# Enderdead/pyNeuralEMPC

Measured on AMD Instinct MI355X. Metric: nlp_callback_evals_per_sec (f + grad f + g + dense jac g), higher is better.
Workload: dtype f64; 1 GPU; configs[1] dims: 2x1 MLP(2x64), H=20, Euler(Discret), fp64; north_star batch=1024 per GPU; batch_per_gpu=1024, H=20, nx=2, nu=1, integrator=discret, n=60, m=40, row_kernel=mfma, parallelism=problem-sharded x1, clock=sustained (timed region after prime_ms of the same step)

## Files before the change

### pyneuralempc_amd/csrc/kernels_coopfx_impl.h

```cpp
#pragma once

#include "kernels_coop_impl.h"
#include "kernels_obj_impl.h"

#ifndef NEMPC_FX_ZERO_EARLY
#define NEMPC_FX_ZERO_EARLY 0
#endif

#ifdef NEMPC_STAMPS_NO_FX
#undef COOP_WGSTAMP
#undef COOP_WGSTAMP_REAL
#define COOP_WGSTAMP(p, i) do { } while (0)
#define COOP_WGSTAMP_REAL(p, i) do { } while (0)
#endif
#ifdef NEMPC_STAMPS_PRO
#define FX_STAMP_PASS(p, i) do { } while (0)
#define FX_STAMP_PRO(p, i) COOP_WGSTAMP(p, i)
#else
#define FX_STAMP_PASS(p, i) COOP_WGSTAMP(p, i)
#define FX_STAMP_PRO(p, i) do { } while (0)
#endif


namespace nempc {

template <typename T, int WP, int NH, int TPW, int NX, int NU>
struct FxLayout {
    static constexpr int MT = WP / 16;
    static constexpr int NIN = NX + NU;
    static constexpr int KS = (NIN + 3) / 4;
    static constexpr int NR = sizeof(T) == 8 ? (NIN + 3) / 4 : 4;
    static constexpr int NRO = sizeof(T) == 8 ? (NX + 3) / 4 : 4;
    static constexpr int JROW = NX * NIN;
    static constexpr int W0F = 0;
    static constexpr int SEED = W0F + KS * MT * 64;
    static constexpr int BIAS = SEED + NX * MT * 16;
    static constexpr int BIASL = BIAS + NH * MT * 16;
    static constexpr int P0 = BIASL + 16;
    static constexpr int SMALL_END = P0 + NIN * MT * 16;
    static constexpr int XH = TPW * MT * 256;
    static constexpr int X = (SMALL_END + 15) & ~15;
    static constexpr int PART = X + 2 * XH;
    static constexpr int PF_SZ = TPW * MT * NX * 16;
    static constexpr int PART_SZ = PF_SZ + NX * TPW * MT * NIN * 16;
    static constexpr int IN_TILE = 16 * (NIN + NX);
    static constexpr int IN = PART + PART_SZ;
    static constexpr int IN_SZ = (TPW * IN_TILE + 15) & ~15;
    static constexpr int TOTAL = IN + 2 * IN_SZ;
};

constexpr int FX_ZCOPY = 512;

struct FxArgs {
    const void* Z;
    const void* X0;
    const void* small;
    const void* wslice;
    int tiles_per_wg, tiles_rem;
    unsigned R;
    unsigned invH;
    int H, n, m;
    int ident;
    int box;
    int small_vecs;
    void* g;
    void* tiles;
    void* jac;
    void* f;
    void* grad;
    const void* P;
    int p_elems;
    int zp_max;
    long long* dbg;
    ObjOffsets oo;
    void* gn_hvals;
    const void* gn_sigma;
    const void* gn_w;
    const int32_t* gn_smap;
    const void* gn_objc;
    int gn_nnz, gn_n_orph;
    void* jac_sp;
    int sp_nnz;
};

constexpr int FX_ARGS_KERNARG_OFFSET = 64;
typedef const FxArgs __attribute__((address_space(4)))* FxArgsK;
__device__ __forceinline__ FxArgsK fx_late_args() {
    const char __attribute__((address_space(4)))* kp =
        (const char __attribute__((address_space(4)))*)__builtin_amdgcn_kernarg_segment_ptr();
    asm volatile("" : "+s"(kp));
    return (FxArgsK)(kp + FX_ARGS_KERNARG_OFFSET);
}

template <typename T, int WP, int NH, int TPW, int NX, int NU>
struct FxCtx {
    using L = FxLayout<T, WP, NH, TPW, NX, NU>;
    T* lds;
    const T* __restrict__ Z;
    const T* __restrict__ X0;
    unsigned R, invH;
    int H, n;
    bool rev;
    T* jac;
    bool box;
    long long* dbg;
};

template <typename T, int NT, int NTHREADS, int NCOL>
struct FxStage {
    static constexpr int ROWS = NT * 16;
    static constexpr int ITEMS = (NCOL * ROWS + NTHREADS - 1) / NTHREADS;
    T v[ITEMS];
};

template <typename T, int WP, int NH, int TPW, int NX, int NU, int NT>
__device__ __forceinline__ void fx_stage_load(const FxCtx<T, WP, NH, TPW, NX, NU>& cx, int t0, int tid,
                                              FxStage<T, NT, (WP / 16) * 64, NX + NU + NX>& sr) {
    constexpr int NIN = NX + NU, NCOL = NIN + NX, ROWS = NT * 16, NTHREADS = (WP / 16) * 64;
#pragma unroll
    for (int it = 0; it < FxStage<T, NT, NTHREADS, NCOL>::ITEMS; ++it) {
        const int item = tid + it * NTHREADS;
        const int col = item / ROWS, idx = item - col * ROWS;
        T v = T(0);
        const unsigned r = (unsigned)t0 * 16u + (unsigned)idx;
        if (col < NCOL && r < cx.R) {
            const unsigned b = cx.invH ? __umulhi(r, cx.invH) : r;
            const int t = (int)(r - b * (unsigned)cx.H);
            const T* z = cx.Z + (size_t)b * cx.n;
            if (col < NX) v = (t == 0) ? cx.X0[(size_t)b * NX + col] : z[(t - 1) * NX + col];
            else if (col < NIN) v = z[cx.H * NX + t * NU + (col - NX)];
            else v = z[t * NX + (col - NIN)];
        }
        sr.v[it] = v;
    }
}

template <typename T, int WP, int NH, int TPW, int NX, int NU, int NT>
__device__ __forceinline__ void fx_stage_store(T* in, int tid, const FxStage<T, NT, (WP / 16) * 64, NX + NU + NX>& sr) {
    constexpr int NIN = NX + NU, NCOL = NIN + NX, ROWS = NT * 16, NTHREADS = (WP / 16) * 64;
    using L = FxLayout<T, WP, NH, TPW, NX, NU>;
#pragma unroll
    for (int it = 0; it < FxStage<T, NT, NTHREADS, NCOL>::ITEMS; ++it) {
        const int item = tid + it * NTHREADS;
        const int col = item / ROWS, idx = item - col * ROWS;
        if (col < NCOL) {
            T* tile = in + (idx >> 4) * L::IN_TILE;
            if (col < NIN) tile[(idx & 15) * NIN + col] = sr.v[it];
            else tile[16 * NIN + (idx & 15) * NX + (col - NIN)] = sr.v[it];
        }
    }
}

__device__ __forceinline__ double fx_qsum(double s) {
    unsigned lo = (unsigned)__double2loint(s), hi = (unsigned)__double2hiint(s);
    auto l16 = __builtin_amdgcn_permlane16_swap(lo, lo, false, false);
    auto h16 = __builtin_amdgcn_permlane16_swap(hi, hi, false, false);
    s = __hiloint2double((int)h16[0], (int)l16[0]) + __hiloint2double((int)h16[1], (int)l16[1]);
    lo = (unsigned)__double2loint(s); hi = (unsigned)__double2hiint(s);
    auto l32 = __builtin_amdgcn_permlane32_swap(lo, lo, false, false);
    auto h32 = __builtin_amdgcn_permlane32_swap(hi, hi, false, false);
    return __hiloint2double((int)h32[0], (int)l32[0]) + __hiloint2double((int)h32[1], (int)l32[1]);
}
__device__ __forceinline__ float fx_qsum(float s) {
    unsigned v = __float_as_uint(s);
    auto a16 = __builtin_amdgcn_permlane16_swap(v, v, false, false);
    s = __uint_as_float(a16[0]) + __uint_as_float(a16[1]);
    v = __float_as_uint(s);
    auto a32 = __builtin_amdgcn_permlane32_swap(v, v, false, false);
// ... 3 lines not shown
__device__ __forceinline__ double fx_swap16_add(double a, double b) {
    auto l = __builtin_amdgcn_permlane16_swap((unsigned)__double2loint(a), (unsigned)__double2loint(b), false, false);
    auto h = __builtin_amdgcn_permlane16_swap((unsigned)__double2hiint(a), (unsigned)__double2hiint(b), false, false);
    return __hiloint2double((int)h[0], (int)l[0]) + __hiloint2double((int)h[1], (int)l[1]);
}
__device__ __forceinline__ double fx_swap32_add(double a, double b) {
    auto l = __builtin_amdgcn_permlane32_swap((unsigned)__double2loint(a), (unsigned)__double2loint(b), false, false);
    auto h = __builtin_amdgcn_permlane32_swap((unsigned)__double2hiint(a), (unsigned)__double2hiint(b), false, false);
    return __hiloint2double((int)h[0], (int)l[0]) + __hiloint2double((int)h[1], (int)l[1]);
}
__device__ __forceinline__ float fx_swap16_add(float a, float b) {
    auto v = __builtin_amdgcn_permlane16_swap(__float_as_uint(a), __float_as_uint(b), false, false);
    return __uint_as_float(v[0]) + __uint_as_float(v[1]);
}
__device__ __forceinline__ float fx_swap32_add(float a, float b) {
    auto v = __builtin_amdgcn_permlane32_swap(__float_as_uint(a), __float_as_uint(b), false, false);
    return __uint_as_float(v[0]) + __uint_as_float(v[1]);
}
template <typename T, int NV>
__device__ __forceinline__ void fx_rowsums_store(const T (&s)[NV], T* dst, int lane) {
    const int q = lane >> 4;
#pragma unroll
    for (int g = 0; g < NV / 4; ++g)
        dst[g * 64 + lane] = fx_swap32_add(fx_swap16_add(s[4 * g], s[4 * g + 1]), fx_swap16_add(s[4 * g + 2], s[4 * g + 3]));
    constexpr int G = NV / 4, REM = NV % 4;
    if constexpr (REM == 1) {
        const T v = fx_qsum(s[4 * G]);
        if (q == 0) dst[G * 64 + lane] = v;
    } else if constexpr (REM == 2) {
        const T p = fx_swap16_add(s[4 * G], s[4 * G + 1]);
        const T v = fx_swap32_add(p, p);
        if (q < 2) dst[G * 64 + lane] = v;
    } else if constexpr (REM == 3) {
        const T v = fx_swap32_add(fx_swap16_add(s[4 * G], s[4 * G + 1]), fx_swap16_add(s[4 * G + 2], s[4 * G + 2]));
        if (q < 3) dst[G * 64 + lane] = v;
    }
}

template <typename T, int NX, int NTHREADS>
__device__ __forceinline__ void fx_zero_rows(T* o_jac, unsigned r0, int nrows, int n, int H, unsigned invH, bool box, int tid) {
    constexpr int VEC = 16 / (int)sizeof(T);
    typedef T vecT __attribute__((ext_vector_type(VEC)));
    const vecT zero = {};
    const int nvec = n / VEC;
#if defined(NEMPC_EXP_NODENSE) || defined(NEMPC_EXP_NOZERO)
    const int drv = 0;
#else
    const int drv = nrows * NX;
#endif
    auto run = [&](const char* base, int nv) {
        const int full = nv / NTHREADS;
        const int voff = tid * 16;
        for (int k = 0; k < full; ++k) {
#ifdef NEMPC_STAMPS
            base = fx_uniform_ptr(base);
#endif
            asm volatile("global_store_dwordx4 %0, %1, %2 sc0 sc1\n\ts_nop 1" ::"v"(voff), "v"(zero), "s"(base) : "memory");
            base += NTHREADS * 16;
        }
#ifdef NEMPC_STAMPS
        base = fx_uniform_ptr(base);
#endif
        if (tid < nv - full * NTHREADS)
            asm volatile("global_store_dwordx4 %0, %1, %2 sc0 sc1\n\ts_nop 1" ::"v"(voff), "v"(zero), "s"(base) : "memory");
    };
    if (!box) {
        run(fx_uniform_ptr(reinterpret_cast<const char*>(o_jac) + (size_t)r0 * NX * (size_t)n * sizeof(T)), drv * nvec);
    } else {
        const int HNX = H * NX;
        for (int s0 = 0; s0 < drv;) {
            const unsigned r = r0 + (unsigned)(s0 / NX);
            const unsigned b = invH ? __umulhi(r, invH) : r;
            const int k = (int)(r - b * (unsigned)H) * NX;
            const int len = drv - s0 < HNX - k ? drv - s0 : HNX - k;
#pragma unroll
            for (int kind = 0; kind < 2; ++kind)
                run(fx_uniform_ptr(reinterpret_cast<const char*>(o_jac) +
                                   ((size_t)b * (2 * HNX) + (size_t)(kind * HNX + k)) * (size_t)n * sizeof(T)), len * nvec);
            s0 += len;
        }
    }
}

template <typename T, int WP, int NH, int TPW, int NX, int NU, int NT, bool FUSE, int ACT, bool GN = false>
__device__ __forceinline__ void fx_pass(const FxCtx<T, WP, NH, TPW, NX, NU>& cx, const CoopWeights<T, WP, NH>& W,
                                        const T* in, int t0, int tid, int& xsel,
                                        const FxStage<T, TPW, (WP / 16) * 64, NX + NU + NX>& nxt, bool has_next, T* in_next) {
    using Ops = MfmaOps<T>;
    using A = Act<T, ACT>;
    static_assert(ACT != NEMPC_ACT_RUNTIME, "the compiled-shape kernels take a compile-time activation");
    using V4 = typename Ops::V4;
    using L = FxLayout<T, WP, NH, TPW, NX, NU>;
    constexpr int MT = WP / 16, NTHREADS = MT * 64, NIN = NX + NU, KS = L::KS, JROW = L::JROW;
    const int lane = tid & 63, w = tid >> 6;
    const int c = lane & 15, q = lane >> 4;
    T* const lds = cx.lds;
    T* const PART = lds + L::PART;

    V4 a[NH][NT];
    {
        const T* bias = lds + L::BIAS + w * 16;
        V4 b0;
#pragma unroll
        for (int r = 0; r < 4; ++r) b0[r] = bias[r * 4 + q];
#pragma unroll
        for (int j = 0; j < NT; ++j) a[0][j] = b0;
#pragma unroll
        for (int ks = 0; ks < KS; ++ks) {
            const T wfrag = lds[L::W0F + (ks * MT + w) * 64 + lane];
            const int d = 4 * ks + q;
#pragma unroll
            for (int j = 0; j < NT; ++j) {
                const T v = d < NIN ? in[j * L::IN_TILE + c * NIN + d] : T(0);
                a[0][j] = Ops::mma(wfrag, v, a[0][j]);
            }
        }
#pragma unroll
        for (int j = 0; j < NT; ++j)
#pragma unroll
            for (int r = 0; r < 4; ++r) a[0][j][r] = A::f(a[0][j][r]);
    }
    FX_STAMP_PRO(cx.dbg, 10);
#if !NEMPC_FX_ZERO_EARLY
    if constexpr (FUSE) {
        if (cx.jac) {
            const unsigned r0 = (unsigned)t0 * 16u;
            const int nrows = r0 + (unsigned)NT * 16u <= cx.R ? NT * 16 : (int)(cx.R - r0);
            fx_zero_rows<T, NX, NTHREADS>(cx.jac, r0, nrows, cx.n, cx.H, cx.invH, cx.box, tid);
        }
    }
#endif
#pragma unroll
    for (int l = 1; l < NH; ++l) {
        T* X = lds + L::X + (xsel & 1) * L::XH;
        ++xsel;
#pragma unroll
        for (int j = 0; j < NT; ++j)
#pragma unroll
            for (int r = 0; r < 4; ++r) X[((j * MT + w) * 4 + r) * 64 + lane] = a[l - 1][j][r];
        lds_barrier();
        const T* bias = lds + L::BIAS + l * MT * 16 + w * 16;
        V4 b0;
#pragma unroll
        for (int r = 0; r < 4; ++r) b0[r] = bias[r * 4 + q];
#pragma unroll
        for (int j = 0; j < NT; ++j) a[l][j] = b0;
#pragma unroll
        for (int mt = 0; mt < MT; ++mt)
#pragma unroll
            for (int r = 0; r < 4; ++r)
#pragma unroll
                for (int j = 0; j < NT; ++j)
                    a[l][j] = Ops::mma(W.wf[l - 1][mt * 4 + r], X[((j * MT + mt) * 4 + r) * 64 + lane], a[l][j]);
#pragma unroll
        for (int j = 0; j < NT; ++j)
#pragma unroll
            for (int r = 0; r < 4; ++r) a[l][j][r] = A::f(a[l][j][r]);
    }
    FX_STAMP_PRO(cx.dbg, 11);
    V4 wl[NX];
#pragma unroll
    for (int k = 0; k < NX; ++k) {
        const T* seed = lds + L::SEED + k * MT * 16 + w * 16;
#pragma unroll
        for (int r = 0; r < 4; ++r) wl[k][r] = seed[r * 4 + q];
    }
    {
        T sv[NT * NX];
#pragma unroll
        for (int j = 0; j < NT; ++j)
#pragma unroll
            for (int k = 0; k < NX; ++k) {
                T v = a[NH - 1][j][0] * wl[k][0];
#pragma unroll
                for (int r = 1; r < 4; ++r) v = fma(a[NH - 1][j][r], wl[k][r], v);
                sv[j * NX + k] = v;
            }
        fx_rowsums_store<T, NT * NX>(sv, PART + w * (TPW * NX) * 16, lane);
    }
    FX_STAMP_PASS(cx.dbg, 5);
    T* const PJ = PART + L::PF_SZ;
    if (cx.rev) {
#pragma unroll
    for (int l = 0; l < NH; ++l)
#pragma unroll
        for (int j = 0; j < NT; ++j)
#pragma unroll
            for (int r = 0; r < 4; ++r) a[l][j][r] = A::d1(a[l][j][r]);

#pragma unroll
    for (int k = 0; k < NX; ++k) {
        V4 cv[NT];
#pragma unroll
        for (int j = 0; j < NT; ++j) cv[j] = wl[k] * a[NH - 1][j];
#pragma unroll
        for (int l = NH - 1; l >= 1; --l) {
            T* X = lds + L::X + (xsel & 1) * L::XH;
            ++xsel;
#pragma unroll
            for (int j = 0; j < NT; ++j)
#pragma unroll
                for (int r = 0; r < 4; ++r) X[((j * MT + w) * 4 + r) * 64 + lane] = cv[j][r];
            lds_barrier();
            V4 cn[NT];
#pragma unroll
// ... 144 lines not shown
            T f = lds[L::BIASL + rr * 4 + qq];
#pragma unroll
            for (int ww = 0; ww < MT; ++ww) f += PART[(ww * (TPW * NX) + j * NX + i) * 16 + cc];
            const T* tin = in + j * L::IN_TILE;
            const T xp = tin[cc * NIN + i];
            const T xt = tin[16 * NIN + cc * NX + i];
            const T phi = (a_ident ? xp : T(0)) + f;
            const unsigned b = cx.invH ? __umulhi(r, cx.invH) : r;
            const int t = (int)(r - b * (unsigned)cx.H);
            T* gp = o_g + (size_t)b * a_m + t * NX + i;
            gp[0] = phi - xt;
            if (a_box) gp[(size_t)cx.H * NX] = xt;
            if constexpr (FUSE) {
                if (o_jac || o_sp) {
                    const int n = cx.n;
                    T ts[NIN];
#pragma unroll
                    for (int d = 0; d < NIN; ++d) {
                        T v = T(0);
#pragma unroll
                        for (int ww = 0; ww < MT; ++ww) v += PJ[((i * MT + ww) * (TPW * NIN) + j * NIN + d) * 16 + cc];
                        if (a_ident && d == i) v += T(1);
                        ts[d] = v;
                    }
                    if (o_jac) {
                    if (o_tiles) {
#pragma unroll
                        for (int d = 0; d < NIN; ++d) o_tiles[(size_t)r * JROW + i * NIN + d] = ts[d];
                    }
                    T* const row = o_jac + ((size_t)b * a_m + (size_t)(t * NX + i)) * (size_t)n;
                    if (t >= 1) {
                        if constexpr (NX == 2 && sizeof(T) == 8) {
                            fx_store_wt2(row + (t - 1) * NX, ts[0], ts[1]);
                        } else {
#pragma unroll
                            for (int jj = 0; jj < NX; ++jj) fx_store_wt(row + (t - 1) * NX + jj, ts[jj]);
                        }
                    }
                    fx_store_wt(row + t * NX + i, T(-1));
#pragma unroll
                    for (int jj = 0; jj < NU; ++jj) fx_store_wt(row + cx.H * NX + t * NU + jj, ts[NX + jj]);
                    if (a_box) fx_store_wt(row + (size_t)cx.H * NX * (size_t)n + t * NX + i, T(1));
                    }
                    if (o_sp) {
                        constexpr int ROW0 = 1 + NU, ROWT = NX + 1 + NU;
                        T* const sp = o_sp + (size_t)b * sp_nnz;
                        if (t >= 1) {
                            T* const pc = sp + NX * ROW0 + ((t - 1) * NX + i) * ROWT;
                            if constexpr (NX == 2 && NU == 1 && sizeof(T) == 8) {
                                fx_store_wt2(pc, ts[0], ts[1]);
                                fx_store_wt2(pc + 2, T(-1), ts[2]);
                            } else {
#pragma unroll
                                for (int jj = 0; jj < NX; ++jj) pc[jj] = ts[jj];
                                pc[NX] = T(-1);
#pragma unroll
                                for (int jj = 0; jj < NU; ++jj) pc[NX + 1 + jj] = ts[NX + jj];
                            }
                        } else {
                            T* const pc = sp + i * ROW0;
                            if constexpr (NX == 2 && NU == 1 && sizeof(T) == 8) {
                                fx_store_wt2(pc, T(-1), ts[2]);
                            } else {
                                pc[0] = T(-1);
#pragma unroll
                                for (int jj = 0; jj < NU; ++jj) pc[1 + jj] = ts[NX + jj];
                            }
                        }
                        if (a_box) sp[NX * ROW0 + (cx.H - 1) * NX * ROWT + t * NX + i] = T(1);
                    }
                }
            }
        }
    }
    FX_STAMP_PASS(cx.dbg, 8);
    FX_STAMP_PASS(cx.dbg, 11);
    lds_barrier();
    FX_STAMP_PASS(cx.dbg, 12);
}

template <typename T, int WP, int NH, int TPW, int NX, int NU, bool FUSE, int ACT, bool GN = false>
__global__ __launch_bounds__((WP / 16) * 64, 2) void rows_coopfx_kernel(
    const void* pZ, const void* pX0, const void* psmall, const void* pwslice, const void* pP, unsigned ppack, unsigned pR,
    unsigned pinvH, int pH, void* pjac, FxArgs a) {
    struct {
        const void *Z, *X0, *small, *wslice, *P;
        int tiles_per_wg, tiles_rem, zp_max, H, n, p_elems;
        unsigned R, invH;
        ObjOffsets oo;
        long long* dbg;
    } pa;
    pa.Z = pZ; pa.X0 = pX0; pa.small = psmall; pa.wslice = pwslice; pa.P = pP;
    pa.tiles_per_wg = (int)(ppack & 0xffu); pa.tiles_rem = (int)((ppack >> 8) & 0x3ffu);
    pa.zp_max = (int)((ppack >> 18) & 0x3ffu);
#ifdef NEMPC_EXP_NOOBJ
    const bool want_obj = false;
#else
    const bool want_obj = ((ppack >> 28) & 3u) != 0;
#endif
    const bool want_rev = (ppack >> 30) & 1u;
    const bool has_box = (ppack >> 31) & 1u;
    pa.R = pR; pa.invH = pinvH; pa.H = pH; pa.n = pH * (NX + NU);
    pa.oo = obj_offsets(pH, NX, NU);
    pa.p_elems = FUSE ? pa.oo.total : 0;
#ifdef NEMPC_STAMPS
    pa.dbg = a.dbg;
#else
    pa.dbg = nullptr;
    (void)a;
#endif
    COOP_WGSTAMP(pa.dbg, 0);
#if defined(NEMPC_STAMPS) && !defined(NEMPC_STAMPS_NO_FX)
    if (pa.dbg && threadIdx.x == 0 && blockIdx.x < 4096)
        pa.dbg[1024 + blockIdx.x * 16 + 15] = ((long long)__builtin_amdgcn_s_getreg(63508) << 32) | (unsigned)__builtin_amdgcn_s_getreg(63492);
#endif
    using L = FxLayout<T, WP, NH, TPW, NX, NU>;
    constexpr int MT = WP / 16;
    constexpr int NTHREADS = MT * 64;
    constexpr int VEC = 16 / (int)sizeof(T);
    constexpr int NCOL = NX + NU + NX;
    typedef T vecT __attribute__((ext_vector_type(VEC)));
    extern __shared__ __attribute__((aligned(16))) unsigned char lds_raw[];
    T* lds = reinterpret_cast<T*>(lds_raw);

    const int tid = threadIdx.x;
    const int lane = tid & 63, w = tid >> 6;

    FxCtx<T, WP, NH, TPW, NX, NU> cx;
    cx.lds = lds;
    cx.Z = static_cast<const T*>(pa.Z);
    cx.X0 = static_cast<const T*>(pa.X0);
    cx.R = pa.R; cx.invH = pa.invH; cx.H = pa.H; cx.n = pa.n; cx.rev = want_rev;
    cx.jac = FUSE ? static_cast<T*>(pjac) : nullptr;
    cx.box = has_box;

    const int t_begin = blockIdx.x * pa.tiles_per_wg + ((int)blockIdx.x < pa.tiles_rem ? (int)blockIdx.x : pa.tiles_rem);
    const int t_end = t_begin + pa.tiles_per_wg + ((int)blockIdx.x < pa.tiles_rem ? 1 : 0);

    FxStage<T, TPW, NTHREADS, NCOL> sr;
    int t0 = t_begin;
    fx_stage_load<T, WP, NH, TPW, NX, NU, TPW>(cx, t0, tid, sr);
    FX_STAMP_PRO(pa.dbg, 1);
    constexpr int SMALL_VECS = (L::SMALL_END + VEC - 1) / VEC;
    constexpr int SMALL_PER_THREAD = (SMALL_VECS + NTHREADS - 1) / NTHREADS;
    vecT sm[SMALL_PER_THREAD];
    {
        const vecT* __restrict__ gs = static_cast<const vecT*>(pa.small);
#pragma unroll
        for (int u = 0; u < SMALL_PER_THREAD; ++u) {
            const int idx = tid + u * NTHREADS;
            if (idx < SMALL_VECS) sm[u] = gs[idx];
        }
    }
    FX_STAMP_PRO(pa.dbg, 2);
    auto obj_range = [&](int side, unsigned& lo, unsigned& hi, int& nlds) {
        const unsigned half_lo = gridDim.x / 2u, half_hi = gridDim.x - half_lo;
        const unsigned Hh = (unsigned)pa.H;
        const unsigned wg = side == 0 ? blockIdx.x : blockIdx.x + half_hi;
        const bool have = blockIdx.x < half_hi && (side == 0 || blockIdx.x < half_lo);
        const unsigned tb = wg * (unsigned)pa.tiles_per_wg + (wg < (unsigned)pa.tiles_rem ? wg : (unsigned)pa.tiles_rem);
        const unsigned te = tb + (unsigned)pa.tiles_per_wg + (wg < (unsigned)pa.tiles_rem ? 1u : 0u);
        unsigned r_lo = tb * 16u, r_hi = te * 16u;
        if (r_lo > pa.R) r_lo = pa.R;
        if (r_hi > pa.R) r_hi = pa.R;
        lo = pa.invH ? __umulhi(r_lo + Hh - 1, pa.invH) : r_lo;
        hi = have ? (pa.invH ? __umulhi(r_hi + Hh - 1, pa.invH) : r_hi) : lo;
        nlds = (int)(hi - lo) < pa.zp_max ? (int)(hi - lo) : pa.zp_max;
    };
    constexpr int ZV_PER_THREAD = 2;
    T zv[2][ZV_PER_THREAD];
    int zcount[2] = {0, 0};
    if constexpr (FUSE) {
        if (want_obj) {
#pragma unroll
            for (int side = 0; side < 2; ++side) {
                unsigned lo, hi;
                int nl;
                obj_range(side, lo, hi, nl);
                zcount[side] = nl * pa.n;
                const T* __restrict__ zsrc = cx.Z + (size_t)lo * pa.n;
#pragma unroll
                for (int u = 0; u < ZV_PER_THREAD; ++u) {
                    const int idx = tid + u * NTHREADS;
                    zv[side][u] = idx < zcount[side] ? zsrc[idx] : T(0);
                }
            }
        }
    }
    constexpr int PV_PER_THREAD = 2;
    T pv[PV_PER_THREAD];
    if constexpr (FUSE) {
        const T* __restrict__ gp = static_cast<const T*>(pa.P);
#pragma unroll
        for (int u = 0; u < PV_PER_THREAD; ++u) {
            const int idx = tid + u * NTHREADS;
            pv[u] = idx < pa.p_elems ? gp[idx] : T(0);
        }
    }
    FX_STAMP_PRO(pa.dbg, 3);
    constexpr int NFRAG = (NH - 1) * 2 * MT * 4 + 8;
    constexpr int NLOAD = (NFRAG + VEC - 1) / VEC;
    vecT wv[NLOAD];
    {
        const vecT* __restrict__ ws = static_cast<const vecT*>(pa.wslice) + (size_t)w * NLOAD * 64 + lane;
#pragma unroll
        for (int k = 0; k < NLOAD; ++k) wv[k] = ws[k * 64];
    }
    FX_STAMP_PASS(pa.dbg, 1);
    FX_STAMP_PRO(pa.dbg, 4);
    cx.dbg = pa.dbg;
    {
        vecT* ls = reinterpret_cast<vecT*>(lds + L::W0F);
#pragma unroll
        for (int u = 0; u < SMALL_PER_THREAD; ++u) {
            const int idx = tid + u * NTHREADS;
            if (idx < SMALL_VECS) ls[idx] = sm[u];
        }
    }
    FX_STAMP_PRO(pa.dbg, 5);
    if constexpr (FUSE) {
#pragma unroll
        for (int u = 0; u < PV_PER_THREAD; ++u) {
            const int idx = tid + u * NTHREADS;
            if (idx < pa.p_elems) lds[L::TOTAL + idx] = pv[u];
        }
    }
    const int p_pad = (pa.p_elems + 15) & ~15;
    if constexpr (FUSE) {
#pragma unroll
        for (int side = 0; side < 2; ++side)
#pragma unroll
            for (int u = 0; u < ZV_PER_THREAD; ++u) {
                const int idx = tid + u * NTHREADS;
                if (idx < zcount[side]) lds[L::TOTAL + p_pad + side * FX_ZCOPY + idx] = zv[side][u];
            }
    }
    FX_STAMP_PASS(pa.dbg, 2);
    FX_STAMP_PRO(pa.dbg, 6);
    CoopWeights<T, WP, NH> W;
    {
        int f = 0;
#pragma unroll
        for (int l = 1; l < NH; ++l) {
#pragma unroll
            for (int i = 0; i < MT * 4; ++i, ++f) W.wf[l - 1][i] = wv[f / VEC][f % VEC];
#pragma unroll
            for (int i = 0; i < MT * 4; ++i, ++f) W.wb[l - 1][i] = wv[f / VEC][f % VEC];
        }
#pragma unroll
        for (int r = 0; r < 4; ++r, ++f) W.wL[r] = wv[f / VEC][f % VEC];
#pragma unroll
        for (int r = 0; r < 4; ++r, ++f) W.w0b[r] = wv[f / VEC][f % VEC];
    }

    FX_STAMP_PASS(pa.dbg, 3);
    int parity = 0, xsel = 0;
    T* const in_base = lds + L::IN;
    fx_stage_store<T, WP, NH, TPW, NX, NU, TPW>(in_base, tid, sr);
    FX_STAMP_PRO(pa.dbg, 7);
    while (t0 < t_end) {
        const int t_cur = t0;
        const int n_cur = t_end - t0 < TPW ? t_end - t0 : TPW;
        t0 += n_cur;
        const bool more = t0 < t_end;
        if (more) fx_stage_load<T, WP, NH, TPW, NX, NU, TPW>(cx, t0, tid, sr);
#if NEMPC_FX_ZERO_EARLY
        if constexpr (FUSE) {
            if (cx.jac) {
                const unsigned r0 = (unsigned)t_cur * 16u;
                const int nrows = r0 + (unsigned)n_cur * 16u <= pa.R ? n_cur * 16 : (int)(pa.R - r0);
                fx_zero_rows<T, NX, NTHREADS>(cx.jac, r0, nrows, pa.n, pa.H, pa.invH, has_box, tid);
            }
        }
#endif
        lds_barrier();
        FX_STAMP_PASS(pa.dbg, 4);
        FX_STAMP_PRO(pa.dbg, 8);
        FX_STAMP_PRO(pa.dbg, 9);
        const T* in = in_base + parity * L::IN_SZ;
        T* const in_next = in_base + (parity ^ 1) * L::IN_SZ;
        if (n_cur == 1) fx_pass<T, WP, NH, TPW, NX, NU, 1, FUSE, ACT, GN>(cx, W, in, t_cur, tid, xsel, sr, more, in_next);
        if constexpr (TPW >= 2) { if (n_cur == 2) fx_pass<T, WP, NH, TPW, NX, NU, 2, FUSE, ACT, GN>(cx, W, in, t_cur, tid, xsel, sr, more, in_next); }
        if constexpr (TPW >= 3) { if (n_cur == 3) fx_pass<T, WP, NH, TPW, NX, NU, 3, FUSE, ACT, GN>(cx, W, in, t_cur, tid, xsel, sr, more, in_next); }
        parity ^= 1;
    }
    if constexpr (FUSE) {
        if (want_obj && blockIdx.x < gridDim.x - gridDim.x / 2u) {
            const FxArgsK ka = fx_late_args();
            T* const o_f = static_cast<T*>(ka->f);
            T* const o_grad = static_cast<T*>(ka->grad);
            unsigned ob_lo[2], ob_hi[2];
            int ob_n[2];
            obj_range(0, ob_lo[0], ob_hi[0], ob_n[0]);
            obj_range(1, ob_lo[1], ob_hi[1], ob_n[1]);
            const int ntot = ob_n[0] + ob_n[1];
            for (int k = w; k < ntot; k += MT) {
                const int side = k < ob_n[0] ? 0 : 1, kk = k - (side ? ob_n[0] : 0);
                objective_row<T>((int)ob_lo[side] + kk, lane, pa.H, NX, NU, pa.oo, lds + L::TOTAL,
                                 lds + L::TOTAL + p_pad + side * FX_ZCOPY + kk * pa.n, o_f, o_grad);
            }
            if (ob_lo[0] + (unsigned)ob_n[0] < ob_hi[0] || ob_lo[1] + (unsigned)ob_n[1] < ob_hi[1]) {
                if (pa.p_elems > PV_PER_THREAD * NTHREADS) {
                    const T* __restrict__ gp = static_cast<const T*>(pa.P);
                    for (int i = tid + PV_PER_THREAD * NTHREADS; i < pa.p_elems; i += NTHREADS) lds[L::TOTAL + i] = gp[i];
                    __syncthreads();
                }
#pragma unroll
                for (int side = 0; side < 2; ++side)
                    for (unsigned b = ob_lo[side] + (unsigned)ob_n[side] + (unsigned)w; b < ob_hi[side]; b += MT)
                        objective_body<T>((int)b, lane, pa.H, NX, NU, pa.oo, lds + L::TOTAL, cx.Z, o_f, o_grad);
            }
        }
    }
    COOP_WGSTAMP(pa.dbg, 14);
    COOP_WGSTAMP_REAL(pa.dbg, 13);
}

}
```

### pyneuralempc_amd/csrc/kernels_mfma_typed.inc

```
#include <cstdlib>
#include <type_traits>

#include "kernels_coop_impl.h"
#include "kernels_coopfx_impl.h"
#include "kernels_hess_impl.h"
#include "kernels_hesscoop_impl.h"
#include "kernels_hessfx_impl.h"

namespace nempc {

namespace {
constexpr int kAct = NEMPC_ACT;
constexpr int kLdsBudget = 150 * 1024;
constexpr int kLdsBudgetCoop = 160 * 1024;
constexpr int kMaxWaves = 8;
inline int coop_dims_on() { static const int on = env_int("NEMPC_COOP_DIMS", 1); return on; }
inline int hfx_on() { static const int on = env_int("NEMPC_HFX", 1); return on; }

template <typename T, int WP, int NH, int TPW, bool SR = false, int OCC = 2, int NXc = 0, int NUc = 0>
bool try_launch_coop(const MfmaParams& p, hipStream_t s, int* rc) {
    constexpr int MT = WP / 16;
    const int NR = coop_nr<T>(p.nin);
    auto up16 = [](int v) { return (v + 15) & ~15; };
    CoopLayout lay{};
// ... 26 lines not shown
    CoopArgs a{};
    a.Z = p.Z; a.X0 = p.X0; a.extra = p.extra;
    a.small = blob + p.off.coop_small;
    a.wslice = blob + p.off.coop_slices;
    a.tiles_per_wg = gp.tiles_per_wg;
    a.tiles_rem = gp.tiles_rem;
    a.R = (unsigned)R;
    a.invH = p.H == 1 ? 0u : (unsigned)((0x100000000ull + (unsigned)p.H - 1) / (unsigned)p.H);
    a.H = p.H; a.n = p.gk.n; a.nx = p.nx; a.nu = p.nu; a.nin = p.nin; a.ne = p.ne;
    a.small_vecs = (p.off.coop_small_elems + VEC - 1) / VEC;
    a.nload = p.off.coop_nload;
    a.early = (p.gk.w == 1 && (p.nin + p.nx + p.ne) * TPW * 16 <= StageRegs<T, MT, TPW>::ITEMS * MT * 64) ? 1 : 0;
    a.l_w0f = lay.w0f; a.l_tail = lay.w0f + p.ks * MT * 64; a.l_x = lay.x; a.l_xhalf = lay.xhalf; a.l_part = lay.part;
    a.l_scratch = lay.scratch; a.l_rowinfo = lay.rowinfo; a.l_scratch2 = scratch2; a.l_rowinfo2 = rowinfo2;
    for (int l = 0; l < NEMPC_MFMA_MAX_HIDDEN; ++l) a.bias_off[l] = p.off.bias[l] - p.off.seed;
    a.acts = p.acts;
    a.biasL_off = p.off.biasL - p.off.seed;
    a.g = p.g; a.tiles = p.tiles; a.stage_out = p.stage_out; a.dbg = p.dbg;
    a.jac = p.fuse_obj ? nullptr : p.fuse_jac;
    a.sp = p.fuse_obj ? nullptr : p.fuse_sparse;
    a.sp_nnz = p.sp_nnz;
    if (!p.fuse_obj && p.obj && (p.fuse_f || p.fuse_grad)) {
        a.obj_f = p.fuse_f; a.obj_grad = p.fuse_grad; a.obj_P = p.obj; a.oo = p.oo; a.B = p.B;
    }
    a.m = p.m; a.NR = NR; a.jsz = 16 * p.nx * p.nin; a.spt = p.scratch_per_wave;
    a.rk4 = p.kind == NEMPC_RK4 ? 1 : 0;
    a.nstages = a.rk4 ? 4 : 1;
    a.ks = p.ks; a.kind = p.kind; a.box = p.box;
    a.xt_off = 16 * p.nin + 2 * 16 * p.nx + (a.rk4 ? 4 : 1) * a.jsz;
    a.ex_off = a.xt_off + 16 * p.nx;
    a.inv_nin = (65536 + p.nin - 1) / p.nin;
    a.stage_stride = p.stage_stride;
    a.inv32_jrow = (unsigned)((0x100000000ull + (unsigned)(p.nx * p.nin) - 1) / (unsigned)(p.nx * p.nin));
    a.inv32_nx = (unsigned)((0x100000000ull + (unsigned)p.nx - 1) / (unsigned)p.nx);
    a.DT = p.DT;
    a.gk = p.gk;
    hipLaunchKernelGGL(kern, dim3(grid), dim3(MT * 64), bytes, s, a);
    hipError_t e = hipGetLastError();
    *rc = e == hipSuccess ? NEMPC_OK : hip_fail(e, "rows_coop_kernel launch");
    return true;
}

template <typename T, int WP, int NH, int TPW, int NX, int NU, bool FUSE, bool GN = false>
int launch_coopfx(const MfmaParams& p, hipStream_t s) {
    using L = FxLayout<T, WP, NH, TPW, NX, NU>;
    constexpr int MT = WP / 16;
    constexpr int VEC = 16 / (int)sizeof(T);
    const int p_elems = FUSE ? p.oo.total : 0;
    const size_t bytes = (size_t)(L::TOTAL + ((p_elems + 15) & ~15) + (FUSE ? 2 * FX_ZCOPY : 0)) * sizeof(T);
    auto kern = rows_coopfx_kernel<T, WP, NH, TPW, NX, NU, FUSE, kAct, GN>;
    NEMPC_HIP(ensure_dynamic_lds(reinterpret_cast<const void*>(kern), bytes));
    int per_cu = (int)((size_t)kLdsBudgetCoop / bytes);
    if (per_cu > 8 / MT) per_cu = 8 / MT;
    if (per_cu < 1) per_cu = 1;
    const GridPlan gp = plan_grid(p.ntiles, p.num_cus, per_cu);
    const int grid = gp.grid;
    const T* blob = static_cast<const T*>(p.blob);
    FxArgs a{};
    a.Z = p.Z; a.X0 = p.X0;
    a.small = blob + p.off.fx_small;
    a.wslice = blob + p.off.coop_slices;
    a.tiles_per_wg = gp.tiles_per_wg;
    a.tiles_rem = gp.tiles_rem;
    a.R = (unsigned)((size_t)p.B * p.H);
    a.invH = p.H == 1 ? 0u : (unsigned)((0x100000000ull + (unsigned)p.H - 1) / (unsigned)p.H);
    a.H = p.H; a.n = p.gk.n; a.m = p.m;
    a.ident = p.kind == NEMPC_DISCRET ? 1 : 0;
    a.box = p.box;
    a.small_vecs = (p.off.fx_small_elems + VEC - 1) / VEC;
    a.g = p.g; a.tiles = p.tiles;
    a.jac = p.fuse_jac; a.f = p.fuse_f; a.grad = p.fuse_grad; a.P = p.obj; a.p_elems = p_elems; a.oo = p.oo;
    a.jac_sp = FUSE ? p.fuse_sparse : nullptr; a.sp_nnz = p.sp_nnz;
    a.dbg = p.dbg;
    if (GN) {
        a.gn_hvals = p.gn_hvals; a.gn_sigma = p.gn_sigma; a.gn_w = p.gn_w; a.gn_smap = p.gn_smap; a.gn_objc = p.gn_objc;
        a.gn_nnz = p.gn_nnz; a.gn_n_orph = p.gn_n_orph;
    }
    if (FUSE) {
        const int nvec = p.gk.n / VEC;
        a.zp_max = p_elems <= 2 * MT * 64 ? (FX_ZCOPY < 2 * MT * 64 ? FX_ZCOPY : 2 * MT * 64) / p.gk.n : 0;
        if (a.jac && (nvec < 1 || p.gk.n % VEC != 0 || (size_t)(TPW * 16 * NX) * p.gk.n * sizeof(T) >= 0x7fffffffull))
            return NEMPC_EUNSUPPORTED;
    }
    if (a.tiles_per_wg > 0xff || a.tiles_rem > 0x3ff || a.zp_max > 0x3ff || a.n != p.H * (NX + NU)) return NEMPC_EUNSUPPORTED;
    const unsigned pack = (unsigned)a.tiles_per_wg | ((unsigned)a.tiles_rem << 8) | ((unsigned)a.zp_max << 18) |
                          (a.f ? 1u << 28 : 0u) | (a.grad ? 1u << 29 : 0u) | ((a.tiles || a.jac || a.jac_sp || GN) ? 1u << 30 : 0u) |
                          (a.box ? 1u << 31 : 0u);
    hipLaunchKernelGGL(kern, dim3(grid), dim3(MT * 64), bytes, s, a.Z, a.X0, a.small, a.wslice, a.P, pack, a.R, a.invH, a.H,
                       FUSE ? a.jac : nullptr, a);
    NEMPC_HIP(hipGetLastError());
    return NEMPC_OK;
}

template <typename T, int WP, int NH>
constexpr bool coop_fits_registers() {
    return ((NH - 1) * 2 * (WP / 16) * 4 + 8) * (int)(sizeof(T) / 4) <= 144;
}

template <typename T, int WP, int NH>
int launch_shape(const MfmaParams& p, bool allow_coop, hipStream_t s, int* kernel_used) {
    const size_t esz = sizeof(T);
    *kernel_used = 3;
    if constexpr (coop_fits_registers<T, WP, NH>()) {
        constexpr size_t hh_lds = (size_t)(NH - 1) * 2 * (WP / 16) * (WP / 16) * 256 * sizeof(T);
        const bool tile_kernel_resident = hh_lds <= 96 * 1024;
        if (allow_coop && p.stage_out) {
            int rc = NEMPC_OK;
            if constexpr (WP == 128 && NH == 3 && sizeof(T) == 4) {
                if (coop_dims_on() && p.nx == 6 && p.nu == 3 && p.nin == 9 && p.gk.w == 1 &&
                    try_launch_coop<T, WP, NH, 1, true, 2, 6, 3>(p, s, &rc)) {
                    *kernel_used = 2;
                    return rc;
                }
            }
            if (try_launch_coop<T, WP, NH, 1, true>(p, s, &rc)) {
                *kernel_used = 2;
                return rc;
            }
        } else if (allow_coop && !(tile_kernel_resident && p.ntiles > 32 * p.num_cus)) {
            int rc = NEMPC_OK;
            if constexpr (WP <= 64) {
                constexpr int tpw_default = (sizeof(T) == 8 && WP >= 64 && NH >= 2) ? 2 : 3;
                static const int tpw_cap = env_int("NEMPC_COOP_TPW", tpw_default);
#ifdef NEMPC_EXP_OCC3
                if constexpr (sizeof(T) == 8 && WP == 64 && NH == 2) {
                    if (try_launch_coop<T, WP, NH, 1, false, 3>(p, s, &rc)) { *kernel_used = 2; return rc; }
                }
#endif
                if ((tpw_cap >= 3 && try_launch_coop<T, WP, NH, 3>(p, s, &rc)) ||
                    (tpw_cap >= 2 && try_launch_coop<T, WP, NH, 2>(p, s, &rc))) {
                    *kernel_used = 2;
                    return rc;
                }
            }
            if constexpr (WP == 128 && NH == 3 && sizeof(T) == 4) {
                if (coop_dims_on() && p.nx == 6 && p.nu == 3 && p.nin == 9 && p.gk.w == 1 &&
                    try_launch_coop<T, WP, NH, 1, false, 2, 6, 3>(p, s, &rc)) {
                    *kernel_used = 2;
                    return rc;
                }
            }
            if (try_launch_coop<T, WP, NH, 1>(p, s, &rc)) {
                *kernel_used = 2;
                return rc;
            }
        }
    }
    if ((p.fuse_jac || p.fuse_sparse) && !p.fuse_obj) return NEMPC_EUNSUPPORTED;
    const size_t blob_bytes = (size_t)((p.off.total + 1) & ~1) * esz;
    const size_t scratch = (size_t)p.scratch_per_wave * esz;
    constexpr size_t hh_bytes = (size_t)(NH - 1) * 2 * (WP / 16) * (WP / 16) * 256 * sizeof(T);
    if constexpr (hh_bytes <= 96 * 1024) {
        int waves = (p.ntiles + p.num_cus - 1) / p.num_cus;
        waves = waves < 1 ? 1 : (waves > kMaxWaves ? kMaxWaves : waves);
        if (blob_bytes + (size_t)waves * scratch <= (size_t)kLdsBudget) {
            int grid = (p.ntiles + waves - 1) / waves;
            if (grid > p.num_cus) grid = p.num_cus;
            return launch_one<T, WP, NH, true, kMaxWaves, kAct>(p, waves, grid, blob_bytes + waves * scratch, s);
        }
    }
    static const int waves_env = env_int("NEMPC_TILE_WAVES", 4);
    int waves = waves_env < 1 ? 1 : (waves_env > 4 ? 4 : waves_env);
    while (waves > 1 && (size_t)waves * scratch > (size_t)kLdsBudget) waves >>= 1;
    const int grid = (p.ntiles + waves - 1) / waves;
    return launch_one<T, WP, NH, false, 4, kAct>(p, waves, grid, (size_t)waves * scratch, s);
}

template <int WP_, int NH_, int NX_, int NU_>
struct FxShape {
    static constexpr int WP = WP_, NH = NH_, NX = NX_, NU = NU_;
};
// ... 272 lines not shown
```

Before: 64.14 million problem-evals/s.

## Reorder coopfx prologue loads and defer LDS stores into first pass

Result: faster. 66.78 million problem-evals/s, median of 6 (+4.1%).

```diff
diff --git a/pyneuralempc_amd/csrc/kernels_coopfx_impl.h b/pyneuralempc_amd/csrc/kernels_coopfx_impl.h
--- a/pyneuralempc_amd/csrc/kernels_coopfx_impl.h
+++ b/pyneuralempc_amd/csrc/kernels_coopfx_impl.h
@@ -48,6 +48,8 @@
     static constexpr int IN_SZ = (TPW * IN_TILE + 15) & ~15;
     static constexpr int TOTAL = IN + 2 * IN_SZ;
 };
+
+template <bool V> struct FxFlag { static constexpr bool value = V; };
 
 constexpr int FX_ZCOPY = 512;
 
@@ -83,7 +85,18 @@
     int sp_nnz;
 };
 
+constexpr int FX_PJAC_KERNARG_OFFSET = 56;
 constexpr int FX_ARGS_KERNARG_OFFSET = 64;
+template <int I, typename... A>
+constexpr int fx_kernarg_offset(void (*)(A...)) {
+    constexpr int sz[] = {(int)sizeof(A)...}, al[] = {(int)alignof(A)...};
+    int o = 0;
+    for (int k = 0; k <= I; ++k) {
+        o = (o + al[k] - 1) / al[k] * al[k];
+        if (k < I) o += sz[k];
+    }
+    return o;
+}
 typedef const FxArgs __attribute__((address_space(4)))* FxArgsK;
 __device__ __forceinline__ FxArgsK fx_late_args() {
     const char __attribute__((address_space(4)))* kp =
@@ -253,10 +266,11 @@
     }
 }
 
-template <typename T, int WP, int NH, int TPW, int NX, int NU, int NT, bool FUSE, int ACT, bool GN = false>
+template <typename T, int WP, int NH, int TPW, int NX, int NU, int NT, bool FUSE, int ACT, bool GN, bool FIRST, typename Late>
 __device__ __forceinline__ void fx_pass(const FxCtx<T, WP, NH, TPW, NX, NU>& cx, const CoopWeights<T, WP, NH>& W,
                                         const T* in, int t0, int tid, int& xsel,
-                                        const FxStage<T, TPW, (WP / 16) * 64, NX + NU + NX>& nxt, bool has_next, T* in_next) {
+                                        const FxStage<T, TPW, (WP / 16) * 64, NX + NU + NX>& nxt, bool has_next, T* in_next,
+                                        const Late& late) {
     using Ops = MfmaOps<T>;
     using A = Act<T, ACT>;
     static_assert(ACT != NEMPC_ACT_RUNTIME, "the compiled-shape kernels take a compile-time activation");
@@ -292,6 +306,13 @@
             for (int r = 0; r < 4; ++r) a[0][j][r] = A::f(a[0][j][r]);
     }
     FX_STAMP_PRO(cx.dbg, 10);
+    if constexpr (FIRST) {
+#pragma unroll
+        for (int j = 0; j < NT; ++j)
+#pragma unroll
+            for (int r = 0; r < 4; ++r) asm volatile("" : "+v"(a[0][j][r]));
+        late();
+    }
 #if !NEMPC_FX_ZERO_EARLY
     if constexpr (FUSE) {
         if (cx.jac) {
@@ -602,7 +623,7 @@
 template <typename T, int WP, int NH, int TPW, int NX, int NU, bool FUSE, int ACT, bool GN = false>
 __global__ __launch_bounds__((WP / 16) * 64, 2) void rows_coopfx_kernel(
     const void* pZ, const void* pX0, const void* psmall, const void* pwslice, const void* pP, unsigned ppack, unsigned pR,
-    unsigned pinvH, int pH, void* pjac, FxArgs a) {
+    unsigned pinvH, unsigned pHG, void* pjac, FxArgs a) {
     struct {
         const void *Z, *X0, *small, *wslice, *P;
         int tiles_per_wg, tiles_rem, zp_max, H, n, p_elems;
@@ -610,6 +631,18 @@
         ObjOffsets oo;
         long long* dbg;
     } pa;
+    {
+        using Self = decltype(&rows_coopfx_kernel<T, WP, NH, TPW, NX, NU, FUSE, ACT, GN>);
+        static_assert(fx_kernarg_offset<9>(Self(nullptr)) == FX_PJAC_KERNARG_OFFSET, "pjac moved: FX_PJAC_KERNARG_OFFSET");
+        static_assert(fx_kernarg_offset<10>(Self(nullptr)) == FX_ARGS_KERNARG_OFFSET, "FxArgs moved: FX_ARGS_KERNARG_OFFSET");
+    }
+    void* jac_arg = nullptr;
+    if constexpr (FUSE) {
+        const char __attribute__((address_space(4)))* kp =
+            (const char __attribute__((address_space(4)))*)__builtin_amdgcn_kernarg_segment_ptr();
+        jac_arg = *(void* const volatile __attribute__((address_space(4)))*)(kp + FX_PJAC_KERNARG_OFFSET);
+    }
+    (void)pjac;
     pa.Z = pZ; pa.X0 = pX0; pa.small = psmall; pa.wslice = pwslice; pa.P = pP;
     pa.tiles_per_wg = (int)(ppack & 0xffu); pa.tiles_rem = (int)((ppack >> 8) & 0x3ffu);
     pa.zp_max = (int)((ppack >> 18) & 0x3ffu);
@@ -620,6 +653,8 @@
 #endif
     const bool want_rev = (ppack >> 30) & 1u;
     const bool has_box = (ppack >> 31) & 1u;
+    const int pH = (int)(pHG & 0xffffu);
+    const unsigned grid_x = pHG >> 16;
     pa.R = pR; pa.invH = pinvH; pa.H = pH; pa.n = pH * (NX + NU);
     pa.oo = obj_offsets(pH, NX, NU);
     pa.p_elems = FUSE ? pa.oo.total : 0;
@@ -651,7 +686,7 @@
     cx.Z = static_cast<const T*>(pa.Z);
     cx.X0 = static_cast<const T*>(pa.X0);
     cx.R = pa.R; cx.invH = pa.invH; cx.H = pa.H; cx.n = pa.n; cx.rev = want_rev;
-    cx.jac = FUSE ? static_cast<T*>(pjac) : nullptr;
+    cx.jac = FUSE ? static_cast<T*>(jac_arg) : nullptr;
     cx.box = has_box;
 
     const int t_begin = blockIdx.x * pa.tiles_per_wg + ((int)blockIdx.x < pa.tiles_rem ? (int)blockIdx.x : pa.tiles_rem);
@@ -673,8 +708,17 @@
         }
     }
     FX_STAMP_PRO(pa.dbg, 2);
+    constexpr int NFRAG = (NH - 1) * 2 * MT * 4 + 8;
+    constexpr int NLOAD = (NFRAG + VEC - 1) / VEC;
+    vecT wv[NLOAD];
+    {
+        const vecT* __restrict__ ws = static_cast<const vecT*>(pa.wslice) + (size_t)w * NLOAD * 64 + lane;
+#pragma unroll
+        for (int k = 0; k < NLOAD; ++k) wv[k] = ws[k * 64];
+    }
+    FX_STAMP_PRO(pa.dbg, 3);
     auto obj_range = [&](int side, unsigned& lo, unsigned& hi, int& nlds) {
-        const unsigned half_lo = gridDim.x / 2u, half_hi = gridDim.x - half_lo;
+        const unsigned half_lo = grid_x / 2u, half_hi = grid_x - half_lo;
         const unsigned Hh = (unsigned)pa.H;
         const unsigned wg = side == 0 ? blockIdx.x : blockIdx.x + half_hi;
         const bool have = blockIdx.x < half_hi && (side == 0 || blockIdx.x < half_lo);
@@ -687,6 +731,16 @@
         hi = have ? (pa.invH ? __umulhi(r_hi + Hh - 1, pa.invH) : r_hi) : lo;
         nlds = (int)(hi - lo) < pa.zp_max ? (int)(hi - lo) : pa.zp_max;
     };
+    constexpr int PV_PER_THREAD = 2;
+    T pv[PV_PER_THREAD];
+    if constexpr (FUSE) {
+        const T* __restrict__ gp = static_cast<const T*>(pa.P);
+#pragma unroll
+        for (int u = 0; u < PV_PER_THREAD; ++u) {
+            const int idx = tid + u * NTHREADS;
+            pv[u] = idx < pa.p_elems ? gp[idx] : T(0);
+        }
+    }
     constexpr int ZV_PER_THREAD = 2;
     T zv[2][ZV_PER_THREAD];
     int zcount[2] = {0, 0};
@@ -707,25 +761,7 @@
             }
         }
     }
-    constexpr int PV_PER_THREAD = 2;
-    T pv[PV_PER_THREAD];
-    if constexpr (FUSE) {
-        const T* __restrict__ gp = static_cast<const T*>(pa.P);
-#pragma unroll
-        for (int u = 0; u < PV_PER_THREAD; ++u) {
-            const int idx = tid + u * NTHREADS;
-            pv[u] = idx < pa.p_elems ? gp[idx] : T(0);
-        }
-    }
-    FX_STAMP_PRO(pa.dbg, 3);
-    constexpr int NFRAG = (NH - 1) * 2 * MT * 4 + 8;
-    constexpr int NLOAD = (NFRAG + VEC - 1) / VEC;
-    vecT wv[NLOAD];
-    {
-        const vecT* __restrict__ ws = static_cast<const vecT*>(pa.wslice) + (size_t)w * NLOAD * 64 + lane;
-#pragma unroll
-        for (int k = 0; k < NLOAD; ++k) wv[k] = ws[k * 64];
-    }
+    asm volatile("" ::: "memory");
     FX_STAMP_PASS(pa.dbg, 1);
     FX_STAMP_PRO(pa.dbg, 4);
     cx.dbg = pa.dbg;
@@ -738,25 +774,10 @@
         }
     }
     FX_STAMP_PRO(pa.dbg, 5);
-    if constexpr (FUSE) {
-#pragma unroll
-        for (int u = 0; u < PV_PER_THREAD; ++u) {
-            const int idx = tid + u * NTHREADS;
-            if (idx < pa.p_elems) lds[L::TOTAL + idx] = pv[u];
-        }
-    }
-    const int p_pad = (pa.p_elems + 15) & ~15;
-    if constexpr (FUSE) {
-#pragma unroll
-        for (int side = 0; side < 2; ++side)
-#pragma unroll
-            for (int u = 0; u < ZV_PER_THREAD; ++u) {
-                const int idx = tid + u * NTHREADS;
-                if (idx < zcount[side]) lds[L::TOTAL + p_pad + side * FX_ZCOPY + idx] = zv[side][u];
-            }
-    }
     FX_STAMP_PASS(pa.dbg, 2);
-    FX_STAMP_PRO(pa.dbg, 6);
+    T* const in_base = lds + L::IN;
+    fx_stage_store<T, WP, NH, TPW, NX, NU, TPW>(in_base, tid, sr);
+    FX_STAMP_PRO(pa.dbg, 7);
     CoopWeights<T, WP, NH> W;
     {
         int f = 0;
@@ -772,13 +793,40 @@
 #pragma unroll
         for (int r = 0; r < 4; ++r, ++f) W.w0b[r] = wv[f / VEC][f % VEC];
     }
-
+    const int p_pad = (pa.p_elems + 15) & ~15;
+    auto late = [&]() {
+#pragma unroll
+        for (int l = 1; l < NH; ++l)
+#pragma unroll
+            for (int i = 0; i < MT * 4; ++i) {
+                asm volatile("" ::"v"(W.wf[l - 1][i]));
+                asm volatile("" ::"v"(W.wb[l - 1][i]));
+            }
+#pragma unroll
+        for (int r = 0; r < 4; ++r) {
+            asm volatile("" ::"v"(W.wL[r]));
+            asm volatile("" ::"v"(W.w0b[r]));
+        }
+        if constexpr (FUSE) {
+#pragma unroll
+            for (int u = 0; u < PV_PER_THREAD; ++u) {
+                const int idx = tid + u * NTHREADS;
+                if (idx < pa.p_elems) lds[L::TOTAL + idx] = pv[u];
+            }
+#pragma unroll
+            for (int side = 0; side < 2; ++side)
+#pragma unroll
+                for (int u = 0; u < ZV_PER_THREAD; ++u) {
+                    const int idx = tid + u * NTHREADS;
+                    if (idx < zcount[side]) lds[L::TOTAL + p_pad + side * FX_ZCOPY + idx] = zv[side][u];
+                }
+        }
+        FX_STAMP_PRO(pa.dbg, 6);
+    };
     FX_STAMP_PASS(pa.dbg, 3);
     int parity = 0, xsel = 0;
-    T* const in_base = lds + L::IN;
-    fx_stage_store<T, WP, NH, TPW, NX, NU, TPW>(in_base, tid, sr);
-    FX_STAMP_PRO(pa.dbg, 7);
-    while (t0 < t_end) {
+    auto one_pass = [&](auto first_tag) {
+        constexpr bool FIRST = decltype(first_tag)::value;
         const int t_cur = t0;
         const int n_cur = t_end - t0 < TPW ? t_end - t0 : TPW;
         t0 += n_cur;
@@ -796,16 +844,17 @@
         lds_barrier();
         FX_STAMP_PASS(pa.dbg, 4);
         FX_STAMP_PRO(pa.dbg, 8);
-        FX_STAMP_PRO(pa.dbg, 9);
         const T* in = in_base + parity * L::IN_SZ;
         T* const in_next = in_base + (parity ^ 1) * L::IN_SZ;
-        if (n_cur == 1) fx_pass<T, WP, NH, TPW, NX, NU, 1, FUSE, ACT, GN>(cx, W, in, t_cur, tid, xsel, sr, more, in_next);
-        if constexpr (TPW >= 2) { if (n_cur == 2) fx_pass<T, WP, NH, TPW, NX, NU, 2, FUSE, ACT, GN>(cx, W, in, t_cur, tid, xsel, sr, more, in_next); }
-        if constexpr (TPW >= 3) { if (n_cur == 3) fx_pass<T, WP, NH, TPW, NX, NU, 3, FUSE, ACT, GN>(cx, W, in, t_cur, tid, xsel, sr, more, in_next); }
+        if (n_cur == 1) fx_pass<T, WP, NH, TPW, NX, NU, 1, FUSE, ACT, GN, FIRST>(cx, W, in, t_cur, tid, xsel, sr, more, in_next, late);
+        if constexpr (TPW >= 2) { if (n_cur == 2) fx_pass<T, WP, NH, TPW, NX, NU, 2, FUSE, ACT, GN, FIRST>(cx, W, in, t_cur, tid, xsel, sr, more, in_next, late); }
+        if constexpr (TPW >= 3) { if (n_cur == 3) fx_pass<T, WP, NH, TPW, NX, NU, 3, FUSE, ACT, GN, FIRST>(cx, W, in, t_cur, tid, xsel, sr, more, in_next, late); }
         parity ^= 1;
-    }
+    };
+    one_pass(FxFlag<true>{});
+    while (t0 < t_end) one_pass(FxFlag<false>{});
     if constexpr (FUSE) {
-        if (want_obj && blockIdx.x < gridDim.x - gridDim.x / 2u) {
+        if (want_obj && blockIdx.x < grid_x - grid_x / 2u) {
             const FxArgsK ka = fx_late_args();
             T* const o_f = static_cast<T*>(ka->f);
             T* const o_grad = static_cast<T*>(ka->grad);
diff --git a/pyneuralempc_amd/csrc/kernels_mfma_typed.inc b/pyneuralempc_amd/csrc/kernels_mfma_typed.inc
--- a/pyneuralempc_amd/csrc/kernels_mfma_typed.inc
+++ b/pyneuralempc_amd/csrc/kernels_mfma_typed.inc
@@ -132,11 +132,14 @@
         if (a.jac && (nvec < 1 || p.gk.n % VEC != 0 || (size_t)(TPW * 16 * NX) * p.gk.n * sizeof(T) >= 0x7fffffffull))
             return NEMPC_EUNSUPPORTED;
     }
-    if (a.tiles_per_wg > 0xff || a.tiles_rem > 0x3ff || a.zp_max > 0x3ff || a.n != p.H * (NX + NU)) return NEMPC_EUNSUPPORTED;
+    if (a.tiles_per_wg > 0xff || a.tiles_rem > 0x3ff || a.zp_max > 0x3ff || a.n != p.H * (NX + NU) || p.H < 1 || p.H > 0xffff ||
+        grid < 1 || grid > 0xffff)
+        return NEMPC_EUNSUPPORTED;
+    const unsigned hg = (unsigned)p.H | ((unsigned)grid << 16);
     const unsigned pack = (unsigned)a.tiles_per_wg | ((unsigned)a.tiles_rem << 8) | ((unsigned)a.zp_max << 18) |
                           (a.f ? 1u << 28 : 0u) | (a.grad ? 1u << 29 : 0u) | ((a.tiles || a.jac || a.jac_sp || GN) ? 1u << 30 : 0u) |
                           (a.box ? 1u << 31 : 0u);
-    hipLaunchKernelGGL(kern, dim3(grid), dim3(MT * 64), bytes, s, a.Z, a.X0, a.small, a.wslice, a.P, pack, a.R, a.invH, a.H,
+    hipLaunchKernelGGL(kern, dim3(grid), dim3(MT * 64), bytes, s, a.Z, a.X0, a.small, a.wslice, a.P, pack, a.R, a.invH, hg,
                        FUSE ? a.jac : nullptr, a);
     NEMPC_HIP(hipGetLastError());
     return NEMPC_OK;
```
